# KatiaJDL/CenterPoly

Hardware: AMD Instinct MI355X
Metric: inference img/s @2048x1024 DLA-34 (1 GPU) (higher is better)
Workload: dtype f32 I/O; split-bf16 x3 contraction (a*b ~ ah*bh + ah*bl + al*bh on bf16 MFMA, ~2^-16 per product) in the convolutions, the heads and DCNv2; f32 accumulate; 1 GPU; BASELINE config 2: DLA-34 + DCNv2, 1x3x1024x2048 synthetic, 16-vertex cartesian head, K=128, forward + sigmoid + NMS/top-k/decode; parallelism=single

## Files before the change

### centerpoly_amd/_C.py

```python
import ctypes
import os
from ctypes import POINTER, Structure, c_char_p, c_float, c_int32, c_int64, c_size_t, c_void_p

import torch

_HERE = os.path.dirname(os.path.abspath(__file__))
LIB_PATH = os.path.join(_HERE, "csrc", "libcenterpoly_hip.so")

CP_OK = 0
REP = {"cartesian": 0, "polar": 1, "polar_fixed": 2}
HEATMAP_UMICH, HEATMAP_ELLIPSE = 0, 1
L1_PLAIN, L1_POLAR, L1_POLAR_FIXED, L1_RELU20, L1_SMOOTH = 0, 1, 2, 3, 4
DCN_BWD_EXACT_F32, DCN_BWD_NARROW_TILES = 1, 2
DCN_CONTRACTION = {"f32": 0, "bf16x3": 1, "bf16x3_region": 3}


class DcnShape(Structure):
    _fields_ = [(n, c_int32) for n in ("B", "Cin", "H", "W", "Cout", "kh", "kw", "stride", "pad",
                                       "dil", "deformable_groups")]


class TargetShape(Structure):
    _fields_ = [(n, c_int32) for n in ("B", "max_objs", "nbr_points", "num_classes", "out_h", "out_w",
                                       "rep", "no_reorder_flip")]
# ... 89 lines not shown
    "cp_map_pairs": (c_int32, [_P, _P, c_int32, _P, c_int32, c_int32, c_int32, _P, _P]),
    "cp_track_associate": (c_int32, [_P, c_int32, _P, _P, _P, _P, ctypes.c_double, c_int32, c_int32, _P, _P, _P, _P]),
    "cp_track_update": (c_int32, [_P, c_int32, _P, c_int32, c_int32, _P, _P, _P, _P, c_int32, _P, _P, _P]),
    "cp_map_pairs_shifted": (c_int32, [_P, _P, c_int32, _P, c_int32, c_int32, c_int32, _P, _P]),
    "cp_track_predict": (c_int32, [_P, _P, c_int32, c_int32, c_int32, _P, _P]),
    "cp_track_kinematics_workspace_bytes": (c_size_t, [c_int32]),
    "cp_track_kinematics": (c_int32, [_P, c_int32, c_int32, c_int32, _P, _P, _P, c_int32, _P, _P, c_size_t, _P]),
    "cp_rle_encode_workspace_bytes": (c_size_t, [c_int32, c_int32, c_int32, c_int64]),
    "cp_rle_encode": (c_int32, [_P, _P, c_int32, c_int32, c_int32, _P, _P, c_int64, _P, c_int64, _P, _P, _P, c_size_t, _P]),
    "cp_rle_decode_workspace_bytes": (c_size_t, [c_int32, c_int64]),
    "cp_rle_decode": (c_int32, [_P, _P, c_int32, c_int32, c_int32, c_int32, _P, _P, _P, c_size_t, _P]),
    "cp_png_deflate_workspace_bytes": (c_size_t, [c_int32] * 4),
    "cp_png_deflate": (c_int32, [_P, _P, c_int32, c_int32, c_int32, c_int32, _P, _P, c_int64, _P, _P, _P, c_size_t, _P]),
    "cp_boundary_overlaps_workspace_bytes": (c_size_t, [c_int32] * 5),
    "cp_boundary_overlaps": (c_int32, [_P, c_int32, _P, _P, c_int32, c_int32, c_int32, _P, c_int32, _P, _P, _P, _P, _P,
                                       _P, c_size_t, _P]),
    "cp_polydet_post_process": (c_int32, [_P, _P, c_float, c_int32, c_int32, c_int32, _P, _P]),
    "cp_polydet_targets_workspace_bytes": (c_size_t, [POINTER(TargetShape)]),
    "cp_polydet_targets": (c_int32, [POINTER(TargetShape)] + [_P] * 19 + [_P, c_size_t, _P]),
    "cp_polydet_targets_ex": (c_int32, [POINTER(TargetShape), c_int32] + [_P] * 19 + [_P, c_size_t, _P]),
    "cp_polydet_dense_targets": (c_int32, [POINTER(TargetShape), _P, _P, c_size_t, _P, _P, _P]),
    "cp_conv_direct_supported": (c_int32, [c_int32] * 5),
    "cp_conv_direct_wgrad_supported": (c_int32, [c_int32] * 5),
    "cp_conv_direct_wgrad": (c_int32, [_P, _P, _P] + [c_int32] * 8 + [_P]),
    "cp_conv_direct_forward": (c_int32, [_P, _P, _P, _P] + [c_int32] * 9 + [_P]),
    "cp_conv_direct_forward_ex": (c_int32, [_P, _P, _P, _P] + [c_int32] * 10 + [_P]),
    "cp_conv3x3_mfma_supported": (c_int32, [c_int32] * 4),
    "cp_conv3x3_mfma_weight_bytes": (c_size_t, [c_int32] * 2),
    "cp_conv3x3_mfma_prepare": (c_int32, [_P, c_int32, c_int32, c_int32, _P, _P]),
    "cp_conv3x3_mfma_forward": (c_int32, [_P, _P, _P, _P, _P] + [c_int32] * 6 + [_P]),
    "cp_conv_mfma_weight_bytes": (c_size_t, [c_int32] * 3),
    "cp_conv_mfma_prepare": (c_int32, [_P, c_int32, c_int32, c_int32, c_int32, _P, _P]),
    "cp_conv3x3_s2_wgrad_supported": (c_int32, [c_int32] * 4),
    "cp_conv3x3_s2_wgrad": (c_int32, [_P, _P, _P] + [c_int32] * 5 + [_P]),
    "cp_conv7x7_c3_supported": (c_int32, [c_int32] * 4),
    "cp_conv7x7_c3_weight_bytes": (c_size_t, [c_int32]),
    "cp_conv7x7_c3_prepare": (c_int32, [_P, c_int32, _P, _P]),
    "cp_conv7x7_c3_forward": (c_int32, [_P, _P, _P, _P] + [c_int32] * 6 + [_P]),
    "cp_conv_mfma_prepare_blocks": (c_int32, [c_int32] * 3),
    "cp_conv_mfma_prepare_batch": (c_int32, [_P, c_int32, c_int32, _P]),
    "cp_conv_mfma_forward": (c_int32, [_P, _P, c_int32, _P, _P, _P, _P] + [c_int32] * 6 + [_P]),
    "cp_conv_mfma_forward_strided": (c_int32, [_P, _P, c_int32, _P, _P, _P, _P] + [c_int32] * 7 + [_P]),
    "cp_dla_base_pair_supported": (c_int32, [c_int32] * 2),
    "cp_dla_base_pair_forward": (c_int32, [_P] * 6 + [c_int32] * 3 + [_P]),
    "cp_dla_base_trio_supported": (c_int32, [c_int32] * 2),
    "cp_dla_base_trio_forward": (c_int32, [_P] * 8 + [c_int32] * 3 + [_P]),
    "cp_conv_mfma_forward_split": (c_int32, [_P, c_int32, _P, _P, _P, _P] + [c_int32] * 9 + [_P]),
    "cp_activation_split": (c_int32, [_P, _P] + [c_int32] * 4 + [_P]),
    "cp_activation_unsplit": (c_int32, [_P, _P] + [c_int32] * 4 + [_P]),
    "cp_conv1x1_stream_supported": (c_int32, [_P, c_int32, c_int32, c_int32, c_int32]),
    "cp_conv1x1_stream_weight_bytes": (c_size_t, [c_int32] * 2),
    "cp_conv1x1_stream_prepare": (c_int32, [_P, c_int32, c_int32, _P, _P]),
    "cp_conv1x1_stream_forward": (c_int32, [_P, _P, c_int32, _P, _P, _P, _P] + [c_int32] * 5 + [_P]),
    "cp_conv1x1_stream_form": (c_int32, [c_int32] * 5),
    "cp_conv1x1_stream_forward_form": (c_int32, [_P, _P, c_int32, _P, _P, _P, _P] + [c_int32] * 7 + [_P]),
    "cp_conv3x3_stream_supported": (c_int32, [c_int32] * 4),
    "cp_conv3x3_stream_form": (c_int32, [c_int32] * 5),
    "cp_conv3x3_stream_forward": (c_int32, [_P] * 5 + [c_int32] * 6 + [_P]),
    "cp_conv3x3_stream_forward_form": (c_int32, [_P] * 5 + [c_int32] * 8 + [_P]),
    "cp_conv_mfma_input_grad_relu_workspace_bytes": (c_size_t, [c_int32] * 4),
    "cp_conv_mfma_input_grad_relu": (c_int32, [_P] * 5 + [c_int32] * 6 + [_P, c_size_t, _P]),
    "cp_conv3x3_s2_input_grad": (c_int32, [_P, _P, _P, _P] + [c_int32] * 5 + [_P]),
    "cp_conv3x3_mfma_wgrad_supported": (c_int32, [c_int32] * 4),
    "cp_conv3x3_mfma_wgrad": (c_int32, [_P, _P, _P] + [c_int32] * 5 + [_P]),
    "cp_conv_mfma_wgrad": (c_int32, [_P, _P, _P] + [c_int32] * 6 + [_P]),
    "cp_heads_fused_w2_bytes": (c_size_t, [c_int32]),
    "cp_heads_fused_prepare_w2": (c_int32, [_P, c_int32, c_int32, _P, _P]),
    "cp_heads_fused_forward": (c_int32, [_P, _P, _P, _P, _P, _P, _P] + [c_int32] * 6 + [_P]),
    "cp_maxpool2x2_forward": (c_int32, [_P, _P] + [c_int32] * 4 + [_P]),
    "cp_maxpool2x2_backward": (c_int32, [_P, _P, _P] + [c_int32] * 4 + [_P]),
    "cp_conv1x1_act_forward": (c_int32, [_P, c_int64, _P, c_int32, _P, _P, _P, c_int32, c_int32, c_int32, c_int64, _P]),
    "cp_soft_nms": (c_int32, [_P, c_int32, c_int32, c_float, c_float, c_float, c_int32]),
    "cp_soft_nms_device": (c_int32, [_P, c_int32, _P, _P, c_int32, c_float, c_float, c_float, c_int32, _P, _P]),
    "cp_merge_detections_workspace_bytes": (c_size_t, [c_int32] * 4),
    "cp_merge_detections": (c_int32, [_P] + [c_int32] * 6 + [c_float] * 3 + [c_int32, _P, _P, _P, c_size_t, _P]),
    "cp_polygon_overlaps_workspace_bytes": (c_size_t, [c_int32] * 4),
    "cp_polygon_overlaps": (c_int32, [_P] + [c_int32] * 5 + [_P, _P, _P, c_size_t, _P]),
    "cp_merge_detections_mask_workspace_bytes": (c_size_t, [c_int32] * 6),
    "cp_merge_detections_mask": (c_int32, [_P] + [c_int32] * 6 + [c_float] * 3 + [c_int32] * 3 + [_P, _P, _P, c_size_t,
                                                                                                  _P]),
    "cp_polydet_decode_workspace_bytes": (c_size_t, [c_int32] * 5),
    "cp_polydet_decode": (c_int32, [_P, _P, _P, _P] + [c_int32] * 7 + [_P, _P, _P, _P, c_size_t, _P]),
    "cp_polydet_decode_ex": (c_int32, [_P, _P, _P, _P] + [c_int32] * 8 + [_P, _P, _P, _P, c_size_t, _P]),
    "cp_sigmoid_focal_workspace_bytes": (c_size_t, [c_int64]),
    "cp_sigmoid_focal_forward": (c_int32, [_P, _P, c_int64, _P, _P, _P, c_size_t, _P]),
    "cp_sigmoid_focal_backward": (c_int32, [_P, _P, c_int64, _P, _P, _P, _P]),
    "cp_gather_l1_forward": (c_int32, [_P, _P, _P, _P, _P] + [c_int32] * 6 + [c_float, _P, _P]),
    "cp_gather_l1_backward": (c_int32, [_P, _P, _P, _P, _P] + [c_int32] * 6 + [c_float, _P, _P, _P]),
    "cp_mse_workspace_bytes": (c_size_t, []),
    "cp_mse_forward": (c_int32, [_P, _P, c_int64, _P, _P, c_size_t, _P]),
    "cp_mse_backward": (c_int32, [_P, _P, c_int64, _P, _P, _P]),
    "cp_dense_l1_workspace_bytes": (c_size_t, []),
    "cp_dense_l1_forward": (c_int32, [_P, _P, _P, c_int64, c_float, _P, _P, c_size_t, _P]),
    "cp_dense_l1_backward": (c_int32, [_P, _P, _P, c_int64, _P, _P, _P, _P]),
    "cp_poly_iou_order_workspace_bytes": (c_size_t, [c_int32] * 3),
    "cp_poly_iou_order_forward": (c_int32, [_P, _P, _P, _P] + [c_int32] * 6 + [_P, _P, _P, _P,
                                                                               c_size_t, _P]),
    "cp_poly_iou_order_backward": (c_int32, [_P, _P, _P, _P] + [c_int32] * 6 + [_P, _P, _P, _P,
                                                                                c_size_t, _P]),
}

EXPORTS = tuple(_SIGNATURES)


def lib():
    global _lib
# ... 121 lines not shown
```

### centerpoly_amd/csrc/upsample.hip

```cpp
#include "cp_common.h"
#include "dcn_internal.h"

namespace {

typedef float f32x2 __attribute__((ext_vector_type(2)));

template <int F>
__global__ __launch_bounds__(256) void dw_up_kernel(const float* __restrict__ x,
                                                    const float* __restrict__ w,
                                                    const float* __restrict__ skip,
                                                    float* __restrict__ out, int C, int H, int W) {
  constexpr int KS = 2 * F, PAD = F / 2;
  const int Ho = H * F, Wo = W * F;
  const int bc = blockIdx.z;
  const int c = bc % C;
  const int oy = blockIdx.y;
  const int ox0 = (blockIdx.x * 256 + threadIdx.x) * 4;
  if (ox0 >= Wo) return;
  const float* wc = w + (long long)c * KS * KS;
  const float* xc = x + (long long)bc * H * W;
  const int ky0 = (oy + PAD) % F;
  const int iy0 = (oy + PAD - ky0) / F;
  float v[4] = {0.f, 0.f, 0.f, 0.f};
#pragma unroll
  for (int r = 0; r < 2; ++r) {
    const int iy = iy0 - r, ky = ky0 + r * F;
    if (iy < 0 || iy >= H) continue;
#pragma unroll
    for (int q = 0; q < 4; ++q) {
      const int ox = ox0 + q;
      const int kx0 = (ox + PAD) % F;
      const int ix0 = (ox + PAD - kx0) / F;
#pragma unroll
      for (int t = 0; t < 2; ++t) {
        const int ix = ix0 - t, kx = kx0 + t * F;
        if (ix < 0 || ix >= W || ox >= Wo) continue;
        v[q] += xc[iy * W + ix] * wc[ky * KS + kx];
      }
    }
  }
  const long long o = ((long long)bc * Ho + oy) * Wo + ox0;
  if (skip) {
    if (ox0 + 3 < Wo) {
      const f32x4 s = *reinterpret_cast<const f32x4*>(skip + o);
      v[0] += s[0]; v[1] += s[1]; v[2] += s[2]; v[3] += s[3];
    } else {
      for (int q = 0; q < 4 && ox0 + q < Wo; ++q) v[q] += skip[o + q];
    }
  }
  if (ox0 + 3 < Wo) *reinterpret_cast<f32x4*>(out + o) = f32x4{v[0], v[1], v[2], v[3]};
  else
    for (int q = 0; q < 4 && ox0 + q < Wo; ++q) out[o + q] = v[q];
}

// ... 433 lines not shown
      g[1][q] = g[3][q];
    }
  }
  if (!gw) return;
#pragma unroll
  for (int a = 0; a < 4; ++a)
#pragma unroll
    for (int b = 0; b < 4; ++b) red[a * 4 + b][threadIdx.x] = acc[a][b];
  __syncthreads();
  const int tap = threadIdx.x >> 4, seg = threadIdx.x & 15;
  float sum = 0.f;
#pragma unroll
  for (int q = 0; q < 16; ++q) sum += red[tap][seg * 16 + q];
  sum += __shfl_xor(sum, 1);
  sum += __shfl_xor(sum, 2);
  sum += __shfl_xor(sum, 4);
  sum += __shfl_xor(sum, 8);
  if (seg == 0 && sum != 0.f) atomicAdd(&gw[(long long)c * 16 + tap], sum);
}

}

extern "C" int cp_depthwise_up_backward(const float* x, const float* weight, const float* grad_out,
                                        float* grad_x, float* grad_weight, int32_t B, int32_t C,
                                        int32_t H, int32_t W, int32_t f, void* stream) {
  CP_CHECK_ARG(weight && grad_out && B > 0 && C > 0 && H > 0 && W > 0);
  if (f != 2 && f != 4) return CP_EUNSUPPORTED;
  if ((long long)B * C > 65535 || H > 65535 || B > 65535 || C > 65535) return CP_EUNSUPPORTED;
  hipStream_t st = (hipStream_t)stream;
  if (f == 2 && (W & 1) == 0 && (grad_weight ? x != nullptr : true) && (long long)H * W * 16 < 0x7FFFFFF0ll &&
      (H + 4 * UB_R - 1) / (4 * UB_R) <= 65535) {
    const dim3 grid((W / 2 + 63) / 64, (H + 4 * UB_R - 1) / (4 * UB_R), B * C);
    hipLaunchKernelGGL(dw_up2_bwd_kernel, grid, dim3(256), 0, st, grad_weight ? x : grad_out, weight, grad_out, grad_x,
                       grad_weight, C, H, W);
    return cp_launch_status();
  }
  if (grad_x) {
    dim3 grid((W + 255) / 256, H, B * C);
    if (f == 2) hipLaunchKernelGGL(dw_up_bwd_data_kernel<2>, grid, dim3(256), 0, st, grad_out, weight, grad_x, C, H, W);
    else hipLaunchKernelGGL(dw_up_bwd_data_kernel<4>, grid, dim3(256), 0, st, grad_out, weight, grad_x, C, H, W);
  }
  if (grad_weight) {
    CP_CHECK_ARG(x);
    const int rows = 8;
    dim3 grid((H + rows - 1) / rows, C, B);
    if (f == 2) hipLaunchKernelGGL(dw_up_bwd_weight_kernel<2>, grid, dim3(256), 0, st, x, grad_out, grad_weight, C, H, W, rows);
    else hipLaunchKernelGGL(dw_up_bwd_weight_kernel<4>, grid, dim3(256), 0, st, x, grad_out, grad_weight, C, H, W, rows);
  }
  return cp_launch_status();
}

namespace {

__device__ __forceinline__ int argmax4(float a, float b, float c, float d) {
  int k = 0;
  float m = a;
  if (b > m || b != b) { m = b; k = 1; }
  if (c > m || c != c) { m = c; k = 2; }
  if (d > m || d != d) { m = d; k = 3; }
  return k;
}

__global__ __launch_bounds__(256) void up2_add_kernel(const float* __restrict__ a, const float* __restrict__ low,
                                                      float* __restrict__ out, int H, int W, long long planes) {
  const int q = blockIdx.x * 256 + threadIdx.x;
  const int y = blockIdx.y;
  const long long pl = blockIdx.z;
  const int W2 = 2 * W;
  if (4 * q >= W2 || pl >= planes) return;
  const float* lr = low + (pl * H + (y >> 1)) * W + 2 * q;
  const long long o = (pl * 2 * H + y) * W2 + 4 * q;
  if ((W & 1) == 0) {
    const float2 l = *reinterpret_cast<const float2*>(lr);
    const float4 v = *reinterpret_cast<const float4*>(a + o);
    *reinterpret_cast<float4*>(out + o) = make_float4(v.x + l.x, v.y + l.x, v.z + l.y, v.w + l.y);
  } else {
    for (int e = 0; e < 4 && 4 * q + e < W2; ++e) out[o + e] = a[o + e] + lr[e >> 1];
  }
}

__global__ __launch_bounds__(256) void maxpool2_fwd_kernel(const float* __restrict__ x, float* __restrict__ out, int H, int W,
                                                           int Ho, int Wo, long long planes) {
  const int q = blockIdx.x * 256 + threadIdx.x;
  const int y = blockIdx.y;
  const long long pl = blockIdx.z;
  const int xo = 2 * q;
  if (xo >= Wo || pl >= planes) return;
  const float* r0 = x + (pl * H + 2 * y) * W + 2 * xo;
  const float* r1 = r0 + W;
  float* o = out + (pl * Ho + y) * Wo + xo;
  if (xo + 1 < Wo && (W & 3) == 0) {
    const float4 a = *reinterpret_cast<const float4*>(r0), b = *reinterpret_cast<const float4*>(r1);
    const float va[4] = {a.x, a.y, b.x, b.y}, vb[4] = {a.z, a.w, b.z, b.w};
    o[0] = va[argmax4(va[0], va[1], va[2], va[3])];
    o[1] = vb[argmax4(vb[0], vb[1], vb[2], vb[3])];
  } else {
#pragma unroll
    for (int e = 0; e < 2; ++e) {
      if (xo + e < Wo) {
        const float v[4] = {r0[2 * e], r0[2 * e + 1], r1[2 * e], r1[2 * e + 1]};
        o[e] = v[argmax4(v[0], v[1], v[2], v[3])];
      }
    }
  }
}

__global__ __launch_bounds__(256) void maxpool2_bwd_kernel(const float* __restrict__ x, const float* __restrict__ go,
                                                           float* __restrict__ gx, int H, int W, int Ho, int Wo,
                                                           long long planes) {
  const int q = blockIdx.x * 256 + threadIdx.x;
  const int yi = blockIdx.y;
  const long long pl = blockIdx.z;
  if (pl >= planes) return;
  if (yi >= Ho) {
// ... 63 lines not shown
```

### centerpoly_amd/models/networks/pose_dla_dcn.py

```python
import math
import os

import numpy as np
import torch
import torch.nn.functional as F
from torch import nn

from ... import _C
from .DCNv2.dcn_v2 import DCN, conv_bias
from . import conv3x3
from .conv3x3 import conv_infer, conv_raw
from .prepared import prepared, release_inference

HEADS_FUSED = True
CONV_DIRECT_WGRAD = True

BN_MOMENTUM = 0.1


def _bn(c):
    return nn.BatchNorm2d(c, momentum=BN_MOMENTUM)



# ... 166 lines not shown
            y = _conv_direct(x, conv, wb, relu)
        if y is not None:
            return y
    if x.is_cuda:
        y = conv_infer([x], conv, wb[0], wb[1], residual, relu, conv=conv)
        if y is not None:
            return y
    if not x.is_cuda:
        y = F.conv2d(x, wb[0], wb[1], conv.stride, conv.padding, conv.dilation, conv.groups)
        if residual is not None:
            y = y + residual
        return F.relu_(y) if relu else y
    y = F.conv2d(x, wb[0], None, conv.stride, conv.padding, conv.dilation, conv.groups)
    B, C, H, W = y.shape
    if not y.is_contiguous() or (H * W) % 4 != 0 or (residual is not None and not residual.is_contiguous()):
        y = y + wb[1].view(1, -1, 1, 1)
        if residual is not None:
            y = y + residual
        return F.relu_(y) if relu else y
    rc = _C.lib().cp_bias_act_inplace(_C.ptr(y), _C.ptr(wb[1]), _C.ptr(residual), B, C, H * W,
                                      1 if relu else 0, _C.stream())
    _C.check(rc, "cp_bias_act_inplace")
    return y


class _MaxPool2x2Fn(torch.autograd.Function):

    @staticmethod
    def forward(ctx, x):
        B, C, H, W = x.shape
        out = torch.empty((B, C, H // 2, W // 2), dtype=torch.float32, device=x.device)
        _C.check(_C.lib().cp_maxpool2x2_forward(_C.ptr(x), _C.ptr(out), B, C, H, W, _C.stream()), "cp_maxpool2x2_forward")
        ctx.save_for_backward(x)
        return out

    @staticmethod
    def backward(ctx, go):
        (x,) = ctx.saved_tensors
        B, C, H, W = x.shape
        gx = torch.empty_like(x)
        _C.check(_C.lib().cp_maxpool2x2_backward(_C.ptr(x), _C.ptr(go.contiguous()), _C.ptr(gx), B, C, H, W,
                                                 _C.stream()), "cp_maxpool2x2_backward")
        return gx


def downsample2(pool, x):
    if (x.is_cuda and x.dtype == torch.float32 and x.dim() == 4 and pool.kernel_size in (2, (2, 2))
            and pool.stride in (2, (2, 2)) and pool.padding in (0, (0, 0)) and not pool.ceil_mode
            and x.shape[0] * x.shape[1] <= 65535 and x.shape[2] >= 2 and x.shape[3] >= 2):
        return _MaxPool2x2Fn.apply(x.contiguous())
    return pool(x)


class _BiasRelu(torch.autograd.Function):

    @staticmethod
    def forward(ctx, y_raw, bias):
        B, C, H, W = y_raw.shape
        _C.check(_C.lib().cp_bias_act_inplace(_C.ptr(y_raw), _C.ptr(bias), None, B, C, H * W, 1, _C.stream()),
                 "cp_bias_act_inplace")
        ctx.mark_dirty(y_raw)
        ctx.save_for_backward(y_raw)
        return y_raw

    @staticmethod
    def backward(ctx, go):
        (y,) = ctx.saved_tensors
        go = go.contiguous()
        B, C, H, W = y.shape
        g = torch.empty_like(go)
        gb = _C.zeros((C,), y.device)
        _C.check(_C.lib().cp_bias_relu_backward(_C.ptr(y), _C.ptr(go), _C.ptr(g), _C.ptr(gb), B, C, H * W,
                                                _C.stream()), "cp_bias_relu_backward")
        return g, gb


def conv_bias_relu(conv, x):
    if (x.is_cuda and conv.bias is not None and x.dtype == torch.float32 and torch.is_grad_enabled()
            and conv.groups == 1):
        y = conv3x3.conv_bias_act(conv, x, True)
        if y is not None:
            return y
        y = conv_raw(conv, x)
        if y.is_contiguous() and (y.shape[2] * y.shape[3]) % 4 == 0 and y.shape[0] * y.shape[1] <= 65535:
            return _BiasRelu.apply(y, conv.bias)
        return F.relu(y + conv.bias.view(1, -1, 1, 1))
    return F.relu(conv(x))


class _BnAct(torch.autograd.Function):
    @staticmethod
    def forward(ctx, x, weight, bias, residual, running_mean, running_var, momentum, eps, relu):
        L = _C.lib()
        x = x.contiguous()
        res = residual.contiguous() if residual is not None else None
        B, C, H, W = x.shape
        y = torch.empty_like(x)
        mean = torch.empty(C, dtype=torch.float32, device=x.device)
        invstd = torch.empty(C, dtype=torch.float32, device=x.device)
        ws = _C.workspace(L.cp_bn_workspace_bytes(B, C, H * W), x.device)
        rc = L.cp_bn_act_forward_train(_C.ptr(x), _C.ptr(weight), _C.ptr(bias), _C.ptr(res), _C.ptr(y),
                                       _C.ptr(mean), _C.ptr(invstd), _C.ptr(running_mean),
                                       _C.ptr(running_var), momentum, eps, 1 if relu else 0, B, C,
                                       H * W, _C.ptr(ws), ws.numel(), _C.stream())
        _C.check(rc, "cp_bn_act_forward_train")
        recompute = relu and residual is None
# ... 95 lines not shown
            res = xs[0] if self.residual else None
            if xs[0].is_cuda:
                y = conv_infer(list(xs), self.conv, self._folded[0], self._folded[1], res, True, conv=self.conv)
                if y is not None:
                    return y
            return _conv_folded(torch.cat(xs, 1), self.conv, self._folded, relu=True, residual=res)
        y = conv3x3.concat_conv1x1(self.conv, xs) if (self.training and xs[0].is_cuda) else None
        if y is None:
            y = conv_train(self.conv, torch.cat(xs, 1))
        return bn_act(self.bn, y, relu=True, residual=xs[0] if self.residual else None)


class Tree(nn.Module):

    def __init__(self, levels, block, in_channels, out_channels, stride=1, level_root=False,
                 root_dim=0, root_kernel_size=1, dilation=1, root_residual=False):
        super().__init__()
        root_dim = root_dim or 2 * out_channels
        if level_root:
            root_dim += in_channels
        self.levels, self.level_root, self.root_dim = levels, level_root, root_dim
        if levels == 1:
            self.tree1 = block(in_channels, out_channels, stride, dilation=dilation)
            self.tree2 = block(out_channels, out_channels, 1, dilation=dilation)
            self.root = Root(root_dim, out_channels, root_kernel_size, root_residual)
        else:
            kw = dict(root_kernel_size=root_kernel_size, dilation=dilation,
                      root_residual=root_residual)
            self.tree1 = Tree(levels - 1, block, in_channels, out_channels, stride, root_dim=0, **kw)
            self.tree2 = Tree(levels - 1, block, out_channels, out_channels,
                              root_dim=root_dim + out_channels, **kw)
        self.downsample = nn.MaxPool2d(stride, stride=stride) if stride > 1 else None
        self.project = None
        if in_channels != out_channels:
            self.project = nn.Sequential(nn.Conv2d(in_channels, out_channels, 1, 1, bias=False),
                                         _bn(out_channels))
        self.project_is_dead = levels > 1 and self.project is not None
        if self.project_is_dead:
            for prm in self.project.parameters():
                prm.requires_grad_(False)

    def fold(self):
        self._folded = _fold_conv_bn(self.project[0], self.project[1]) if self.project is not None \
            else None

    share_pool = True

    def _same_pool(self, other):
        a, b = self.downsample, getattr(other, "downsample", None)
        return isinstance(other, Tree) and a is not None and b is not None and \
            (a.kernel_size, a.stride, a.padding, a.dilation, a.ceil_mode) == \
            (b.kernel_size, b.stride, b.padding, b.dilation, b.ceil_mode)

    def forward(self, x, residual=None, children=None, bottom=None):
        children = [] if children is None else children
        if bottom is None:
            bottom = x if self.downsample is None else downsample2(self.downsample, x)
        if self.project is None:
            residual = bottom
        elif self.project_is_dead:
            residual = None
            if self.training:
                with torch.no_grad():
                    if bottom.is_cuda:
                        bn_act(self.project[1], conv_train(self.project[0], bottom), relu=False)
                    else:
                        self.project(bottom)
        elif _use_folded(self):
            residual = _conv_folded(bottom, self.project[0], self._folded)
        else:
            residual = bn_act(self.project[1], conv_train(self.project[0], bottom), relu=False)
        if self.level_root:
            children.append(bottom)
        if Tree.share_pool and self.levels > 1 and not torch.is_grad_enabled() and self._same_pool(self.tree1):
            x1 = self.tree1(x, residual, bottom=bottom)
        else:
            x1 = self.tree1(x, residual)
        if self.levels == 1:
            return self.root(self.tree2(x1), x1, *children)
        children.append(x1)
        return self.tree2(x1, children=children)


class DLA(nn.Module):
    def __init__(self, levels, channels, num_classes=1000, block=BasicBlock, residual_root=False,
                 linear_root=False):
        super().__init__()
        self.channels, self.num_classes = channels, num_classes
        c = channels
        self.base_layer = nn.Sequential(nn.Conv2d(3, c[0], 7, 1, 3, bias=False), _bn(c[0]),
                                        nn.ReLU(inplace=True))
        self.level0 = self._conv_level(c[0], c[0], levels[0])
        self.level1 = self._conv_level(c[0], c[1], levels[1], stride=2)
        for i in range(2, 6):
            setattr(self, "level%d" % i, Tree(levels[i], block, c[i - 1], c[i], 2,
                                              level_root=i > 2, root_residual=residual_root))

    @staticmethod
    def _conv_level(inplanes, planes, convs, stride=1, dilation=1):
        mods = []
        for i in range(convs):
            mods += [nn.Conv2d(inplanes, planes, 3, stride if i == 0 else 1, dilation, dilation,
                               bias=False), _bn(planes), nn.ReLU(inplace=True)]
            inplanes = planes
        return nn.Sequential(*mods)

    def fold(self):
        seqs = (self.base_layer, self.level0, self.level1)
        if any(len(seq) != 3 for seq in seqs):
            self._folded = None
            return
        self._folded = [_fold_conv_bn(seq[0], seq[1]) for seq in seqs]

    def forward(self, x):
        pyramid = []
        if _use_folded(self):
            skip0 = getattr(self, "skip_level0_output", False)
            y1 = _base_trio(self, x) if skip0 else None
            if y1 is None:
                x = _conv_folded(x, self.base_layer[0], self._folded[0], relu=True)
                y1 = _base_pair(self, x) if skip0 else None
            if y1 is not None:
                pyramid += [None, y1]
                x = y1
            else:
                for seq, wb in zip((self.level0, self.level1), self._folded[1:]):
                    x = _conv_folded(x, seq[0], wb, relu=True)
# ... 369 lines not shown
```

### include/centerpoly_hip.h

```cpp
#ifndef CENTERPOLY_HIP_H
#define CENTERPOLY_HIP_H

#include <stddef.h>
#include <stdint.h>

#ifdef __cplusplus
extern "C" {
#endif

#define CP_ABI_VERSION 3

enum {
  CP_OK = 0,
  CP_EINVAL = -1,
  CP_EUNSUPPORTED = -2,
  CP_EWORKSPACE = -3,
  CP_EHIP = -4
};


enum { CP_REP_CARTESIAN = 0, CP_REP_POLAR = 1, CP_REP_POLAR_FIXED = 2 };

enum {
  CP_DCN_F32 = 0,
// ... 82 lines not shown
int cp_conv_direct_supported(int32_t Cin, int32_t Cout, int32_t k, int32_t stride, int32_t pad);
int cp_conv_direct_forward(const float* x, const float* w, const float* bias, float* out, int32_t B, int32_t Cin,
                           int32_t H, int32_t W, int32_t Cout, int32_t k, int32_t stride, int32_t pad,
                           int32_t relu, void* stream);
int cp_conv_direct_forward_ex(const float* x, const float* w, const float* bias, float* out, int32_t B, int32_t Cin,
                           int32_t H, int32_t W, int32_t Cout, int32_t k, int32_t stride, int32_t pad,
                           int32_t relu, int32_t split_bf16, void* stream);

int cp_conv3x3_mfma_supported(int32_t Cin, int32_t Cout, int32_t H, int32_t W);
size_t cp_conv3x3_mfma_weight_bytes(int32_t Cin, int32_t Cout);
int cp_conv3x3_mfma_prepare(const float* weight, int32_t Cin, int32_t Cout, int32_t transposed, void* wperm,
                            void* stream);
int cp_conv3x3_mfma_forward(const float* x, const void* wperm, const float* bias, const float* residual, float* out,
                            int32_t B, int32_t Cin, int32_t H, int32_t W, int32_t Cout, int32_t relu, void* stream);

size_t cp_conv_mfma_weight_bytes(int32_t Cin, int32_t Cout, int32_t taps);
int cp_conv_mfma_prepare(const float* weight, int32_t Cin, int32_t Cout, int32_t taps, int32_t transposed, void* wperm,
                         void* stream);
typedef struct cp_conv_prepare_job {
  const float* weight;
  void* wperm;
  int32_t Cin, Cout, taps, transposed, first_block, reserved;
} cp_conv_prepare_job;
int32_t cp_conv_mfma_prepare_blocks(int32_t Cin, int32_t Cout, int32_t taps);
int cp_conv_mfma_prepare_batch(const cp_conv_prepare_job* jobs_device, int32_t njobs, int32_t total_blocks, void* stream);
int cp_conv_mfma_forward(const float* const* xs, const int32_t* cs, int32_t nsrc, const void* wperm, const float* bias,
                         const float* residual, float* out, int32_t B, int32_t H, int32_t W, int32_t Cout,
                         int32_t taps, int32_t relu, void* stream);
int cp_conv_mfma_forward_strided(const float* const* xs, const int32_t* cs, int32_t nsrc, const void* wperm,
                                 const float* bias, const float* residual, float* out, int32_t B, int32_t H, int32_t W,
                                 int32_t Cout, int32_t taps, int32_t stride, int32_t relu, void* stream);
int cp_dla_base_pair_supported(int32_t H, int32_t W);
int cp_dla_base_pair_forward(const float* x, const float* w0, const float* b0, const float* w1, const float* b1, float* out,
                             int32_t B, int32_t H, int32_t W, void* stream);
int cp_dla_base_trio_supported(int32_t H, int32_t W);
int cp_dla_base_trio_forward(const float* image, const void* stem_wperm, const float* stem_bias, const float* w0,
                             const float* b0, const float* w1, const float* b1, float* out, int32_t B, int32_t H,
                             int32_t W, void* stream);
int cp_conv_mfma_forward_split(const void* x, int32_t x_split, const void* wperm, const float* bias, const float* residual,
                               void* out, int32_t out_split, int32_t B, int32_t Cin, int32_t H, int32_t W, int32_t Cout,
                               int32_t taps, int32_t stride, int32_t relu, void* stream);
int cp_activation_split(const float* x, void* out, int32_t B, int32_t C, int32_t H, int32_t W, void* stream);
int cp_activation_unsplit(const void* in, float* x, int32_t B, int32_t C, int32_t H, int32_t W, void* stream);
int cp_conv1x1_stream_supported(const int32_t* cs, int32_t nsrc, int32_t Cout, int32_t H, int32_t W);
size_t cp_conv1x1_stream_weight_bytes(int32_t Cin, int32_t Cout);
int cp_conv1x1_stream_prepare(const float* weight, int32_t Cin, int32_t Cout, void* wperm, void* stream);
int cp_conv1x1_stream_forward(const float* const* xs, const int32_t* cs, int32_t nsrc, const void* wperm, const float* bias,
                              const float* residual, float* out, int32_t B, int32_t H, int32_t W, int32_t Cout,
                              int32_t relu, void* stream);
int cp_conv1x1_stream_form(int32_t Cin, int32_t Cout, int32_t H, int32_t W, int32_t B);
int cp_conv1x1_stream_forward_form(const float* const* xs, const int32_t* cs, int32_t nsrc, const void* wperm,
                                   const float* bias, const float* residual, float* out, int32_t B, int32_t H, int32_t W,
                                   int32_t Cout, int32_t relu, int32_t nb, int32_t ks, void* stream);
int cp_conv3x3_stream_supported(int32_t Cin, int32_t Cout, int32_t H, int32_t W);
int cp_conv3x3_stream_form(int32_t Cin, int32_t Cout, int32_t H, int32_t W, int32_t B);
int cp_conv3x3_stream_forward(const float* x, const void* wperm, const float* bias, const float* residual, float* out,
                              int32_t B, int32_t Cin, int32_t H, int32_t W, int32_t Cout, int32_t relu, void* stream);
int cp_conv3x3_stream_forward_form(const float* x, const void* wperm, const float* bias, const float* residual, float* out,
                                   int32_t B, int32_t Cin, int32_t H, int32_t W, int32_t Cout, int32_t relu, int32_t nt,
                                   int32_t ks, void* stream);
int cp_conv3x3_s2_wgrad_supported(int32_t Cin, int32_t Cout, int32_t H, int32_t W);
int cp_conv3x3_s2_wgrad(const float* x, const float* grad_out, float* gw, int32_t B, int32_t Cin, int32_t H, int32_t W,
                        int32_t Cout, void* stream);

int cp_conv7x7_c3_supported(int32_t Cout, int32_t H, int32_t W, int32_t stride);
size_t cp_conv7x7_c3_weight_bytes(int32_t Cout);
int cp_conv7x7_c3_prepare(const float* weight, int32_t Cout, void* wperm, void* stream);
int cp_conv7x7_c3_forward(const float* x, const void* wperm, const float* bias, float* out, int32_t B, int32_t H,
                          int32_t W, int32_t Cout, int32_t stride, int32_t relu, void* stream);

size_t cp_conv_mfma_input_grad_relu_workspace_bytes(int32_t B, int32_t Cin, int32_t H, int32_t W);
int cp_conv_mfma_input_grad_relu(const float* grad_out, const void* wperm_t, const float* y, float* grad_y,
                                 float* grad_bias, int32_t B, int32_t Cin, int32_t H, int32_t W, int32_t Cout,
                                 int32_t taps, void* workspace, size_t workspace_bytes, void* stream);
int cp_conv3x3_s2_input_grad(const float* grad_out, const void* wperm_t, const float* residual, float* grad_in, int32_t B,
                             int32_t Cin, int32_t H, int32_t W, int32_t Cout, void* stream);

int cp_conv3x3_mfma_wgrad_supported(int32_t Cin, int32_t Cout, int32_t H, int32_t W);
int cp_conv3x3_mfma_wgrad(const float* x, const float* go, float* gw, int32_t B, int32_t Cin, int32_t H, int32_t W,
                          int32_t Cout, void* stream);
int cp_conv_mfma_wgrad(const float* x, const float* go, float* gw, int32_t B, int32_t Cin, int32_t H, int32_t W,
                       int32_t Cout, int32_t taps, void* stream);

int cp_conv_direct_wgrad_supported(int32_t Cin, int32_t Cout, int32_t k, int32_t stride, int32_t pad);
int cp_conv_direct_wgrad(const float* x, const float* go, float* gw, int32_t B, int32_t Cin, int32_t H, int32_t W,
                         int32_t Cout, int32_t k, int32_t stride, int32_t pad, void* stream);

size_t cp_heads_fused_w2_bytes(int32_t head_conv);
int cp_heads_fused_prepare_w2(const float* w2, int32_t cout, int32_t head_conv, void* w2perm, void* stream);
int cp_heads_fused_forward(const float* x, const void* wperm1, const float* b1, const void* const* w2perm,
                           const float* const* b2, float* const* out, const int32_t* cout, int32_t nheads, int32_t B,
                           int32_t Cin, int32_t H, int32_t W, int32_t head_conv, void* stream);

int cp_conv1x1_act_forward(const float* y, int64_t y_bstride, const float* in_bias, int32_t relu_in,
                           const float* w_t, const float* bias, float* out, int32_t B, int32_t Cin,
                           int32_t Cout, int64_t HW, void* stream);

int cp_instance_masks(const int32_t* poly, const uint8_t* flags, int32_t n, int32_t N, int32_t H, int32_t W,
                      uint8_t* masks, int32_t* counts, void* stream);

int cp_id_histogram(const uint16_t* ids, int32_t H, int32_t W, int32_t* hist, void* stream);
size_t cp_instance_overlaps_workspace_bytes(int32_t n, int32_t G, int32_t H, int32_t W);
int cp_instance_overlaps(const uint8_t* masks, int32_t n, const uint16_t* gt_ids, int32_t H, int32_t W,
                         const int32_t* inst_ids, int32_t G, const int32_t* void_ids, int32_t V, int32_t* inter,
                         int32_t* void_inter, int32_t* pred_pixels, void* workspace, size_t workspace_bytes,
                         void* stream);
// ... 248 lines not shown
```

Before: 396.7 img/s.

## Fuse 2x2 maxpool with tree projection 1x1 conv at DLA tree entry

Measured after the change: 397.8 img/s (median of 3 runs). Within noise of the previous version (+0.3%).

```diff
diff --git a/centerpoly_amd/_C.py b/centerpoly_amd/_C.py
--- a/centerpoly_amd/_C.py
+++ b/centerpoly_amd/_C.py
@@ -165,6 +165,9 @@
     "cp_conv1x1_stream_weight_bytes": (c_size_t, [c_int32] * 2),
     "cp_conv1x1_stream_prepare": (c_int32, [_P, c_int32, c_int32, _P, _P]),
     "cp_conv1x1_stream_forward": (c_int32, [_P, _P, c_int32, _P, _P, _P, _P] + [c_int32] * 5 + [_P]),
+    "cp_pool2_conv1x1_stream_supported": (c_int32, [c_int32] * 4),
+    "cp_pool2_conv1x1_stream_forward": (c_int32, [_P] * 5 + [c_int32] * 5 + [_P]),
+    "cp_pool2_conv1x1_stream_forward_form": (c_int32, [_P] * 5 + [c_int32] * 7 + [_P]),
     "cp_conv1x1_stream_form": (c_int32, [c_int32] * 5),
     "cp_conv1x1_stream_forward_form": (c_int32, [_P, _P, c_int32, _P, _P, _P, _P] + [c_int32] * 7 + [_P]),
     "cp_conv3x3_stream_supported": (c_int32, [c_int32] * 4),
diff --git a/centerpoly_amd/csrc/maxpool2.h b/centerpoly_amd/csrc/maxpool2.h
--- /dev/null
+++ b/centerpoly_amd/csrc/maxpool2.h
@@ -0,0 +1,11 @@
+#pragma once
+#include <hip/hip_runtime.h>
+
+__device__ __forceinline__ int argmax4(float a, float b, float c, float d) {
+  int k = 0;
+  float m = a;
+  if (b > m || b != b) { m = b; k = 1; }
+  if (c > m || c != c) { m = c; k = 2; }
+  if (d > m || d != d) { m = d; k = 3; }
+  return k;
+}
diff --git a/centerpoly_amd/csrc/pool_conv_stream.hip b/centerpoly_amd/csrc/pool_conv_stream.hip
--- /dev/null
+++ b/centerpoly_amd/csrc/pool_conv_stream.hip
@@ -0,0 +1,273 @@
+#include <type_traits>
+
+#include "cp_common.h"
+#include "maxpool2.h"
+
+namespace {
+
+typedef __bf16 bf16x8 __attribute__((ext_vector_type(8)));
+typedef __bf16 bf16x2 __attribute__((ext_vector_type(2)));
+typedef float f32x2 __attribute__((ext_vector_type(2)));
+typedef unsigned u32x2 __attribute__((ext_vector_type(2)));
+typedef unsigned u32x4 __attribute__((ext_vector_type(4)));
+
+constexpr int KC = 32;
+constexpr int CB = 64;
+constexpr int MT = CB / 16;
+constexpr unsigned OOB = 0x80000000u;
+
+struct PoolArgs {
+  const float* x;
+  const bf16x8* wp;
+  const float* bias;
+  float* bottom;
+  float* out;
+  int Cin, Cout, H, W, Wo, HWo, nchunk, ncb, vec;
+};
+
+__device__ __forceinline__ void split2(float v0, float v1, unsigned& hi, unsigned& lo) {
+  const bf16x2 h = __builtin_convertvector(f32x2{v0, v1}, bf16x2);
+  const unsigned hb = __builtin_bit_cast(unsigned, h);
+  const float h0 = __builtin_bit_cast(float, hb << 16), h1 = __builtin_bit_cast(float, hb & 0xffff0000u);
+  const bf16x2 l = __builtin_convertvector(f32x2{v0 - h0, v1 - h1}, bf16x2);
+  hi = hb;
+  lo = __builtin_bit_cast(unsigned, l);
+}
+
+template <int NT, int KS, int DEPTH, bool BOT>
+__global__ __launch_bounds__(256, 2) void pool2_conv1x1_stream_kernel(PoolArgs a) {
+  constexpr int PG = 4 / KS;
+  const int lane = threadIdx.x & 63;
+  const int wave = __builtin_amdgcn_readfirstlane(threadIdx.x >> 6);
+  const int q = wave % KS, grp = wave / KS;
+  const int c = lane & 15, g = lane >> 4;
+  int lw = blockIdx.x;
+  if ((gridDim.x & 7) == 0) lw = (blockIdx.x & 7) * (gridDim.x >> 3) + (blockIdx.x >> 3);
+  const int cb = lw % a.ncb, pg = (lw / a.ncb) * PG + grp, b = blockIdx.y;
+  const int HWo = a.HWo, P0 = pg * 16 * NT;
+  const unsigned iplane = (unsigned)(a.H * a.W) * 4u, oplane = (unsigned)HWo * 4u, rowb = (unsigned)a.W * 4u;
+
+  unsigned vin[NT], vbot[NT];
+#pragma unroll
+  for (int n = 0; n < NT; ++n) {
+    const int p = P0 + 16 * n + c;
+    const unsigned y = (unsigned)p / (unsigned)a.Wo, x = (unsigned)p - y * (unsigned)a.Wo;
+    const bool in = p < HWo;
+    vin[n] = in ? (unsigned)(8 * g) * iplane + (2u * y * (unsigned)a.W + 2u * x) * 4u : OOB;
+    vbot[n] = (BOT && in && cb == 0) ? (unsigned)(8 * g) * oplane + (unsigned)p * 4u : OOB;
+  }
+
+  const __amdgpu_buffer_rsrc_t rs_x = __builtin_amdgcn_make_buffer_rsrc(
+      const_cast<float*>(a.x + (long long)b * a.Cin * a.H * a.W), 0, (int)((unsigned)a.Cin * iplane), 0x00020000);
+  const __amdgpu_buffer_rsrc_t rs_bot = __builtin_amdgcn_make_buffer_rsrc(
+      BOT ? a.bottom + (long long)b * a.Cin * HWo : a.out, 0, BOT ? (int)((unsigned)a.Cin * oplane) : 0, 0x00020000);
+
+  const long long tstride = (long long)a.nchunk * 128;
+  const bf16x8* wq = a.wp + (long long)cb * MT * tstride + lane;
+  const int nmine = a.nchunk > q ? (a.nchunk - q + KS - 1) / KS : 0;
+
+  auto issue_x = [&](int i, u32x2 (&r)[NT][8][2]) __attribute__((always_inline)) {
+    const bool live = i < nmine;
+    const int cc = live ? (q + i * KS) * KC : 0;
+#pragma unroll
+    for (int n = 0; n < NT; ++n) {
+      const unsigned vo = live ? vin[n] : OOB;
+#pragma unroll
+      for (int j = 0; j < 8; ++j) {
+        r[n][j][0] = __builtin_amdgcn_raw_buffer_load_b64(rs_x, vo, (unsigned)(cc + j) * iplane, 0);
+        r[n][j][1] = __builtin_amdgcn_raw_buffer_load_b64(rs_x, vo + rowb, (unsigned)(cc + j) * iplane, 0);
+      }
+    }
+  };
+  auto issue_w = [&](int i, bf16x8 (&w)[MT][2]) __attribute__((always_inline)) {
+    const bf16x8* wsrc = wq + (long long)min(q + i * KS, a.nchunk - 1) * 128;
+#pragma unroll
+    for (int m = 0; m < MT; ++m) {
+      w[m][0] = wsrc[m * tstride];
+      w[m][1] = wsrc[m * tstride + 64];
+    }
+  };
+
+  f32x4 acc[MT][NT];
+#pragma unroll
+  for (int m = 0; m < MT; ++m)
+#pragma unroll
+    for (int n = 0; n < NT; ++n) acc[m][n] = f32x4{0.f, 0.f, 0.f, 0.f};
+
+  u32x2 r[DEPTH][NT][8][2];
+  bf16x8 w[DEPTH][MT][2];
+#pragma unroll
+  for (int d = 0; d < DEPTH; ++d) {
+    issue_x(d, r[d]);
+    __builtin_amdgcn_sched_barrier(0);
+    issue_w(d, w[d]);
+    __builtin_amdgcn_sched_barrier(0);
+  }
+
+  for (int i = 0; i < nmine; i += DEPTH) {
+#pragma unroll
+    for (int d = 0; d < DEPTH; ++d) {
+      const bool live = i + d < nmine;
+      const int cc = live ? (q + (i + d) * KS) * KC : 0;
+      bf16x8 xh[NT], xl[NT];
+#pragma unroll
+      for (int n = 0; n < NT; ++n) {
+        float v[8];
+#pragma unroll
+        for (int j = 0; j < 8; ++j) {
+          const unsigned u[4] = {r[d][n][j][0][0], r[d][n][j][0][1], r[d][n][j][1][0], r[d][n][j][1][1]};
+          const float win[4] = {__builtin_bit_cast(float, u[0]), __builtin_bit_cast(float, u[1]),
+                                __builtin_bit_cast(float, u[2]), __builtin_bit_cast(float, u[3])};
+          v[j] = win[argmax4(win[0], win[1], win[2], win[3])];
+        }
+        if constexpr (BOT) {
+          const unsigned vo = live ? vbot[n] : OOB;
+#pragma unroll
+          for (int j = 0; j < 8; ++j)
+            __builtin_amdgcn_raw_buffer_store_b32(__builtin_bit_cast(unsigned, v[j]), rs_bot, vo, (unsigned)(cc + j) * oplane, 0);
+        }
+        unsigned hi[4], lo[4];
+#pragma unroll
+        for (int j = 0; j < 4; ++j) split2(v[2 * j], v[2 * j + 1], hi[j], lo[j]);
+        xh[n] = __builtin_bit_cast(bf16x8, hi);
+        xl[n] = __builtin_bit_cast(bf16x8, lo);
+      }
+      issue_x(i + d + DEPTH, r[d]);
+      __builtin_amdgcn_sched_barrier(0);
+#pragma unroll
+      for (int m = 0; m < MT; ++m)
+#pragma unroll
+        for (int n = 0; n < NT; ++n) {
+          acc[m][n] = __builtin_amdgcn_mfma_f32_16x16x32_bf16(xh[n], w[d][m][0], acc[m][n], 0, 0, 0);
+          acc[m][n] = __builtin_amdgcn_mfma_f32_16x16x32_bf16(xl[n], w[d][m][0], acc[m][n], 0, 0, 0);
+          acc[m][n] = __builtin_amdgcn_mfma_f32_16x16x32_bf16(xh[n], w[d][m][1], acc[m][n], 0, 0, 0);
+        }
+      __builtin_amdgcn_sched_barrier(0);
+      issue_w(i + d + DEPTH, w[d]);
+    }
+  }
+
+  constexpr int NTILE = MT * NT;
+  const __amdgpu_buffer_rsrc_t rs_o = __builtin_amdgcn_make_buffer_rsrc(a.out + (long long)b * a.Cout * HWo, 0,
+                                                                        (int)((unsigned)a.Cout * oplane), 0x00020000);
+  const __amdgpu_buffer_rsrc_t rs_b =
+      __builtin_amdgcn_make_buffer_rsrc(const_cast<float*>(a.bias), 0, a.bias ? a.Cout * 4 : 0, 0x00020000);
+  __shared__ f32x4 red[KS > 1 ? 4 * NTILE * 64 : 1];
+  auto finish = [&](auto wide) __attribute__((always_inline)) {
+    constexpr bool VEC = decltype(wide)::value;
+    float bv[MT];
+    unsigned off[MT][NT];
+#pragma unroll
+    for (int m = 0; m < MT; ++m) {
+      const int co = cb * CB + m * 16 + c;
+      bv[m] = __builtin_bit_cast(float, __builtin_amdgcn_raw_buffer_load_b32(rs_b, (unsigned)co * 4u, 0, 0));
+#pragma unroll
+      for (int n = 0; n < NT; ++n) {
+        const int p = P0 + 16 * n + 4 * g;
+        const bool mine = KS == 1 || (m * NT + n) % KS == q;
+        off[m][n] = (mine && co < a.Cout && p < HWo) ? ((unsigned)co * (unsigned)HWo + (unsigned)p) * 4u : OOB;
+      }
+    }
+    if constexpr (KS > 1) {
+#pragma unroll
+      for (int m = 0; m < MT; ++m)
+#pragma unroll
+        for (int n = 0; n < NT; ++n) red[(wave * NTILE + m * NT + n) * 64 + lane] = acc[m][n];
+      __syncthreads();
+    }
+#pragma unroll
+    for (int m = 0; m < MT; ++m)
+#pragma unroll
+      for (int n = 0; n < NT; ++n) {
+        const int t = m * NT + n;
+        if (KS > 1 && t % KS != q) continue;
+        f32x4 s = acc[m][n];
+        if constexpr (KS > 1) {
+          s = red[((grp * KS + 0) * NTILE + t) * 64 + lane];
+#pragma unroll
+          for (int k = 1; k < KS; ++k) s += red[((grp * KS + k) * NTILE + t) * 64 + lane];
+        }
+        f32x4 o;
+#pragma unroll
+        for (int r = 0; r < 4; ++r) o[r] = s[r] + bv[m];
+        if constexpr (VEC) {
+          __builtin_amdgcn_raw_buffer_store_b128(__builtin_bit_cast(u32x4, o), rs_o, off[m][n], 0, 0);
+        } else {
+          const int p = P0 + 16 * n + 4 * g;
+#pragma unroll
+          for (int r = 0; r < 4; ++r)
+            __builtin_amdgcn_raw_buffer_store_b32(__builtin_bit_cast(unsigned, (float)o[r]), rs_o,
+                                                  (off[m][n] != OOB && p + r < HWo) ? off[m][n] + 4u * r : OOB, 0, 0);
+        }
+      }
+  };
+  if (a.vec) finish(std::true_type{});
+  else finish(std::false_type{});
+}
+
+bool shape_ok(int32_t Cin, int32_t Cout, int32_t H, int32_t W) {
+  if (Cin < KC || Cin % KC || Cout < CB || Cout % CB || H < 2 || W < 2 || (H & 1) || (W & 1)) return false;
+  const long long HW = (long long)H * W, HWo = HW / 4;
+  if (Cin * HW * 4 >= (1ll << 31) || Cout * HWo * 4 >= (1ll << 31)) return false;
+  if (((HWo + 15) / 16) * (Cout / CB) >= (1ll << 31) || Cin >= (1 << 20)) return false;
+  return true;
+}
+
+}
+
+int cp_pool2_conv1x1_stream_supported(int32_t Cin, int32_t Cout, int32_t H, int32_t W) {
+  return shape_ok(Cin, Cout, H, W) ? 1 : 0;
+}
+
+int cp_pool2_conv1x1_stream_forward_form(const float* x, const void* wperm, const float* bias, float* bottom, float* out,
+                                         int32_t B, int32_t Cin, int32_t H, int32_t W, int32_t Cout, int32_t nb, int32_t ks,
+                                         void* stream) {
+  CP_CHECK_ARG(x && wperm && out && B >= 1 && Cin >= 1 && H >= 1 && W >= 1 && Cout >= 1);
+  if (!shape_ok(Cin, Cout, H, W) || B > 65535) return CP_EUNSUPPORTED;
+  if (reinterpret_cast<unsigned long long>(x) & 7) return CP_EUNSUPPORTED;
+  PoolArgs a;
+  a.x = x;
+  a.wp = (const bf16x8*)wperm;
+  a.bias = bias;
+  a.bottom = bottom;
+  a.out = out;
+  a.Cin = Cin;
+  a.Cout = Cout;
+  a.H = H;
+  a.W = W;
+  a.Wo = W / 2;
+  a.HWo = (H / 2) * (W / 2);
+  a.nchunk = Cin / KC;
+  a.ncb = Cout / CB;
+  a.vec = (a.HWo & 3) == 0 && (reinterpret_cast<unsigned long long>(out) & 15) == 0;
+  if (nb == 0 && ks == 0) {
+    ks = cp_conv1x1_stream_form(Cin, Cout, H / 2, W / 2, B) & 255;
+    nb = 2;
+  }
+  if ((nb != 1 && nb != 2) || (ks != 1 && ks != 2 && ks != 4)) return CP_EINVAL;
+  const auto launch = [&](auto kernel) {
+    const unsigned npg = (unsigned)((a.HWo + 16 * nb - 1) / (16 * nb));
+    const unsigned pgw = 4 / ks;
+    hipLaunchKernelGGL(kernel, dim3(((npg + pgw - 1) / pgw) * a.ncb, B), dim3(256), 0, (hipStream_t)stream, a);
+  };
+  const auto pick = [&](auto bot) {
+    constexpr bool BOT = decltype(bot)::value;
+    if (nb == 2) {
+      if (ks == 1) launch(pool2_conv1x1_stream_kernel<2, 1, 1, BOT>);
+      else if (ks == 2) launch(pool2_conv1x1_stream_kernel<2, 2, 1, BOT>);
+      else launch(pool2_conv1x1_stream_kernel<2, 4, 1, BOT>);
+    } else {
+      if (ks == 1) launch(pool2_conv1x1_stream_kernel<1, 1, 2, BOT>);
+      else if (ks == 2) launch(pool2_conv1x1_stream_kernel<1, 2, 2, BOT>);
+      else launch(pool2_conv1x1_stream_kernel<1, 4, 2, BOT>);
+    }
+  };
+  if (bottom) pick(std::true_type{});
+  else pick(std::false_type{});
+  return cp_launch_status();
+}
+
+int cp_pool2_conv1x1_stream_forward(const float* x, const void* wperm, const float* bias, float* bottom, float* out,
+                                    int32_t B, int32_t Cin, int32_t H, int32_t W, int32_t Cout, void* stream) {
+  return cp_pool2_conv1x1_stream_forward_form(x, wperm, bias, bottom, out, B, Cin, H, W, Cout, 0, 0, stream);
+}
diff --git a/centerpoly_amd/csrc/upsample.hip b/centerpoly_amd/csrc/upsample.hip
--- a/centerpoly_amd/csrc/upsample.hip
+++ b/centerpoly_amd/csrc/upsample.hip
@@ -1,5 +1,6 @@
 #include "cp_common.h"
 #include "dcn_internal.h"
+#include "maxpool2.h"
 
 namespace {
 
@@ -539,14 +540,6 @@
 
 namespace {
 
-__device__ __forceinline__ int argmax4(float a, float b, float c, float d) {
-  int k = 0;
-  float m = a;
-  if (b > m || b != b) { m = b; k = 1; }
-  if (c > m || c != c) { m = c; k = 2; }
-  if (d > m || d != d) { m = d; k = 3; }
-  return k;
-}
 
 __global__ __launch_bounds__(256) void up2_add_kernel(const float* __restrict__ a, const float* __restrict__ low,
                                                       float* __restrict__ out, int H, int W, long long planes) {
diff --git a/centerpoly_amd/models/networks/pose_dla_dcn.py b/centerpoly_amd/models/networks/pose_dla_dcn.py
--- a/centerpoly_amd/models/networks/pose_dla_dcn.py
+++ b/centerpoly_amd/models/networks/pose_dla_dcn.py
@@ -242,6 +242,47 @@
     return pool(x)
 
 
+TREE_ENTRY = "auto"
+
+_TREE_ENTRY_SHAPES = frozenset([(32, 64, 512 * 1024), (64, 128, 256 * 512)])
+
+
+def _tree_entry(x, pool, tree, want_bottom):
+    if TREE_ENTRY == "off" or tree.project is None or tree.project_is_dead or not _use_folded(tree):
+        return None
+    conv = tree.project[0]
+    if not (x.is_cuda and x.dtype == torch.float32 and x.dim() == 4 and conv3x3.mfma_enabled()
+            and isinstance(pool, nn.MaxPool2d) and pool.kernel_size in (2, (2, 2)) and pool.stride in (2, (2, 2))
+            and pool.padding in (0, (0, 0)) and pool.dilation in (1, (1, 1)) and not pool.ceil_mode
+            and (conv.kernel_size, conv.stride, conv.padding, conv.dilation, conv.groups)
+            == ((1, 1), (1, 1), (0, 0), (1, 1), 1)):
+        return None
+    w, bias = tree._folded
+    B, cin, H, W = x.shape
+    cout = w.shape[0]
+    if cin != w.shape[1] or B > 65535 or not (TREE_ENTRY == "force" or (cin, cout, H * W) in _TREE_ENTRY_SHAPES):
+        return None
+    L = _C.lib()
+    if not L.cp_pool2_conv1x1_stream_supported(cin, cout, H, W):
+        return None
+    wp, _ = prepared(conv, "conv", (w,), lambda: conv3x3._permute(w.contiguous(), cin, cout, 0))
+    x = x.contiguous()
+    out = torch.empty((B, cout, H // 2, W // 2), dtype=torch.float32, device=x.device)
+    bottom = torch.empty((B, cin, H // 2, W // 2), dtype=torch.float32, device=x.device) if want_bottom else None
+    key = ("tree_entry", cin, cout, H, W, B)
+    end = _C.kernel_timer.start(key) if _C.kernel_timer is not None else None
+    rc = L.cp_pool2_conv1x1_stream_forward(_C.ptr(x), _C.ptr(wp), _C.ptr(bias), _C.ptr(bottom), _C.ptr(out), B, cin, H, W,
+                                           cout, _C.stream())
+    if rc == -2:
+        if end is not None:
+            _C.kernel_timer.drop(key, end)
+        return None
+    _C.check(rc, "cp_pool2_conv1x1_stream_forward")
+    if end is not None:
+        end.record()
+    return bottom, out
+
+
 class _BiasRelu(torch.autograd.Function):
 
     @staticmethod
@@ -443,11 +484,24 @@
             (a.kernel_size, a.stride, a.padding, a.dilation, a.ceil_mode) == \
             (b.kernel_size, b.stride, b.padding, b.dilation, b.ceil_mode)
 
-    def forward(self, x, residual=None, children=None, bottom=None):
+    def forward(self, x, residual=None, children=None, bottom=None, projected=False):
         children = [] if children is None else children
-        if bottom is None:
+        share = Tree.share_pool and self.levels > 1 and not torch.is_grad_enabled() and self._same_pool(self.tree1)
+        entry = None
+        if bottom is None and not projected and self.downsample is not None:
+            if self.levels == 1:
+                entry = _tree_entry(x, self.downsample, self, self.level_root)
+            elif share and self.tree1.levels == 1:
+                entry = _tree_entry(x, self.downsample, self.tree1, True)
+        if entry is not None:
+            bottom = entry[0]
+        elif bottom is None:
             bottom = x if self.downsample is None else downsample2(self.downsample, x)
-        if self.project is None:
+        if projected:
+            pass
+        elif entry is not None and self.levels == 1:
+            residual = entry[1]
+        elif self.project is None:
             residual = bottom
         elif self.project_is_dead:
             residual = None
@@ -463,7 +517,9 @@
             residual = bn_act(self.project[1], conv_train(self.project[0], bottom), relu=False)
         if self.level_root:
             children.append(bottom)
-        if Tree.share_pool and self.levels > 1 and not torch.is_grad_enabled() and self._same_pool(self.tree1):
+        if entry is not None and self.levels > 1:
+            x1 = self.tree1(x, entry[1], bottom=bottom, projected=True)
+        elif share:
             x1 = self.tree1(x, residual, bottom=bottom)
         else:
             x1 = self.tree1(x, residual)
diff --git a/include/centerpoly_hip.h b/include/centerpoly_hip.h
--- a/include/centerpoly_hip.h
+++ b/include/centerpoly_hip.h
@@ -158,6 +158,12 @@
 int cp_conv1x1_stream_forward_form(const float* const* xs, const int32_t* cs, int32_t nsrc, const void* wperm,
                                    const float* bias, const float* residual, float* out, int32_t B, int32_t H, int32_t W,
                                    int32_t Cout, int32_t relu, int32_t nb, int32_t ks, void* stream);
+int cp_pool2_conv1x1_stream_supported(int32_t Cin, int32_t Cout, int32_t H, int32_t W);
+int cp_pool2_conv1x1_stream_forward(const float* x, const void* wperm, const float* bias, float* bottom_or_null, float* out,
+                                    int32_t B, int32_t Cin, int32_t H, int32_t W, int32_t Cout, void* stream);
+int cp_pool2_conv1x1_stream_forward_form(const float* x, const void* wperm, const float* bias, float* bottom_or_null,
+                                         float* out, int32_t B, int32_t Cin, int32_t H, int32_t W, int32_t Cout, int32_t nb,
+                                         int32_t ks, void* stream);
 int cp_conv3x3_stream_supported(int32_t Cin, int32_t Cout, int32_t H, int32_t W);
 int cp_conv3x3_stream_form(int32_t Cin, int32_t Cout, int32_t H, int32_t W, int32_t B);
 int cp_conv3x3_stream_forward(const float* x, const void* wperm, const float* bias, const float* residual, float* out,
```
